# gotaku6629/CTC

Hardware: AMD Instinct MI355X
Metric: ctc_samples_per_sec (higher is better)
Workload: dtype f32; 1 GPU; NoBlankCTC B=256 T=150 C=158 S<=20 fp32 (BASELINE configs[1]); variant=noblank, per_gpu_batch=256, global_batch=256, T=150, C=158, S=20, parallelism=dp1 (batch-sharded), launch=graph, graph_steps=50, step=fused loss+grad launch + scale_grad launch (loss.backward(), grad_out=1)

## Files before the change

### ctc_amd/csrc/noblank_r16.hpp

```cpp
#pragma once

namespace ctc {

typedef float f2_t __attribute__((ext_vector_type(2)));

#define CTC_ROW16(OP)                                                                   \
    "s_nop 1\n\t" OP " %0, %0, %0 quad_perm:[1,0,3,2] row_mask:0xf bank_mask:0xf\n\t"   \
    "s_nop 1\n\t" OP " %0, %0, %0 quad_perm:[2,3,0,1] row_mask:0xf bank_mask:0xf\n\t"   \
    "s_nop 1\n\t" OP " %0, %0, %0 row_half_mirror row_mask:0xf bank_mask:0xf\n\t"       \
    "s_nop 1\n\t" OP " %0, %0, %0 row_mirror row_mask:0xf bank_mask:0xf\n\t"            \
    "s_nop 1"
__device__ __forceinline__ void row16_allmax(float &v) { asm volatile(CTC_ROW16("v_max_f32_dpp") : "+v"(v)); }
__device__ __forceinline__ void row16_allsum(float &v) { asm volatile(CTC_ROW16("v_add_f32_dpp") : "+v"(v)); }
__device__ __forceinline__ void row16_allmax(int &v) { asm volatile(CTC_ROW16("v_max_i32_dpp") : "+v"(v)); }

constexpr int kR16Pad = 2 * kPrefetch + 1;
#ifndef CTC_R16_BLOCK
#define CTC_R16_BLOCK 16
#endif
constexpr int kR16Block = CTC_R16_BLOCK;
__host__ __device__ inline int r16_pitch(int T)
{
    int tp = T + 2 * kR16Pad + 1;
    while ((tp & 3) != 2) ++tp;
    return tp;
}

__device__ __forceinline__ int r16_row(int T, int u, int g, int k)
{
    const int H = (T + 1) >> 1, idx = 2 * kPipeWorkers * g + 2 * u + (k >> 1);
    if ((k & 1) == 0) return idx < H ? idx : -1;
    return idx < T - H ? T - 1 - idx : -1;
}

struct R16Smem {
    int TP;
    cell_t *em, *al, *be;
    float *dummy, *stage, *cs;
    int *cnt, *lab, *occ, *done;
    __device__ R16Smem(float *base, int T, int SP, int RP)
    {
        TP = r16_pitch(T);
        cell_t *lat = reinterpret_cast<cell_t *>(base);
        em = lat + kR16Pad;
        al = em + (size_t)(SP + 1) * TP;
        be = al + (size_t)(SP + 1) * TP;
        dummy = reinterpret_cast<float *>(lat + (size_t)3 * (SP + 1) * TP);
        cnt = reinterpret_cast<int *>(dummy + 8);
        lab = cnt + 16;
        occ = lab + ((SP + 3) & ~3);
        cs = reinterpret_cast<float *>(occ + ((SP + 3) & ~3) + 4);
        done = reinterpret_cast<int *>(cs + 4 * kPipeWorkers);
        stage = cs + 64;
    }
};

static size_t r16_smem_bytes(int T, int SP, int C)
{
    const int RP = 32 * ((C + 31) / 32);
    return (size_t)3 * (SP + 1) * r16_pitch(T) * 8 + (8 + 16 + 2 * ((SP + 3) & ~3) + 4 + 64) * 4 +
           (size_t)kPipeWorkers * 4 * RP * 4;
}

template <bool FWD>
__device__ __forceinline__ cell_t r16_chain(const NoblankParams &p, const R16Smem &sm, int T, int Tb, int L, int SP, const int lane)
{
    constexpr int G = kPipeRows / 4;
    constexpr int D = FWD ? 1 : -1;
    const int lrow = lane < SP ? lane : SP;
    const cell_t *erow = sm.em + (size_t)lrow * sm.TP;
    cell_t *orow = (FWD ? sm.al : sm.be) + (size_t)lrow * sm.TP;
    typedef float pair_t __attribute__((ext_vector_type(4)));
    float m;
    int k;

    const int H = (T + 1) >> 1;
    const int pos0 = FWD ? 0 : T - Tb;
    const int own = FWD ? H : T - H;
    typedef const volatile __attribute__((address_space(3))) int lds_cvint;
    const int *cp = sm.cnt + (lane < kPipeWorkers ? lane : 0);
    int have = 0;
    bool starved = false;
    auto wait_upto = [&](int i_last) {
        const int q = pos0 + (i_last < Tb ? i_last : Tb - 1);
        int ng = q / (2 * kPipeWorkers) + 1;
        if (q >= own || ng > G) ng = G;
        if (ng <= have) return;
        const int need = lane < kPipeWorkers ? 4 * ng : 0;
        int spins = 0;
        while (__builtin_amdgcn_ballot_w64(*(lds_cvint *)cp < need) != 0) {
            if (++spins >= kSpinLimit) { starved = true; break; }
            __builtin_amdgcn_s_sleep(1);
        }
        lds_order();
        have = ng;
    };
#define CTC_R16_STEP_ASM(K, M, EM, EK, K2, T2, DPP)                                                  \
            "v_max_i32_dpp %[kk], " K ", " K " " DPP "\n\t"                                           \
            "v_add_u32 " K2 ", %[kk], " EK "\n\t"                                                     \
            "v_sub_u32 %[d1], " K ", %[kk]\n\t"                                                       \
            "v_sub_u32_dpp %[d2], " K ", %[kk] " DPP "\n\t"                                           \
            "v_ldexp_f32 %[d1], " EM ", %[d1]\n\t"                                                    \
            "v_ldexp_f32 %[d2], " EM ", %[d2]\n\t"                                                    \
            "v_mul_f32 " T2 ", " M ", %[d1]\n\t"                                                      \
            "v_fmac_f32_dpp " T2 ", " M ", %[d2] " DPP "\n\t"
#ifdef CTC_X_ROWDPP
#define CTC_R16_DPP_F "row_shr:1 row_mask:0xf bank_mask:0xf bound_ctrl:1"
#define CTC_R16_DPP_B "row_shl:1 row_mask:0xf bank_mask:0xf bound_ctrl:1"
#else
#define CTC_R16_DPP_F "wave_shr:1 row_mask:0xf bank_mask:0xf bound_ctrl:1"
#define CTC_R16_DPP_B "wave_shl:1 row_mask:0xf bank_mask:0xf bound_ctrl:1"
#endif
    auto step = [&](float em_, float ek_) {
        int kk, k2, d1, d2;
        float t;
        if (FWD)
            asm("s_nop 1\n\t" CTC_R16_STEP_ASM("%[k]", "%[m]", "%[em]", "%[ek]", "%[k2]", "%[t]", CTC_R16_DPP_F)
                : [kk] "=&v"(kk), [k2] "=&v"(k2), [d1] "=&v"(d1), [d2] "=&v"(d2), [t] "=&v"(t)
                : [k] "v"(k), [m] "v"(m), [em] "v"(em_), [ek] "v"(ek_));
        else
            asm("s_nop 1\n\t" CTC_R16_STEP_ASM("%[k]", "%[m]", "%[em]", "%[ek]", "%[k2]", "%[t]", CTC_R16_DPP_B)
                : [kk] "=&v"(kk), [k2] "=&v"(k2), [d1] "=&v"(d1), [d2] "=&v"(d2), [t] "=&v"(t)
                : [k] "v"(k), [m] "v"(m), [em] "v"(em_), [ek] "v"(ek_));
        m = t;
        k = k2;
    };
    auto step2 = [&](pair_t e, bool first) {
        const float e1m = FWD ? e.x : e.z, e1k = FWD ? e.y : e.w, e2m = FWD ? e.z : e.x, e2k = FWD ? e.w : e.y;
        int kk, d1, d2, k1, k2;
        float m1, m2;
#define CTC_R16_PAIR(NOP, DPP)                                                                       \
        asm(NOP CTC_R16_STEP_ASM("%[k]", "%[m]", "%[e1m]", "%[e1k]", "%[k1]", "%[m1]", DPP)           \
                CTC_R16_STEP_ASM("%[k1]", "%[m1]", "%[e2m]", "%[e2k]", "%[k2]", "%[m2]", DPP)         \
            : [kk] "=&v"(kk), [d1] "=&v"(d1), [d2] "=&v"(d2), [k1] "=&v"(k1), [k2] "=&v"(k2),        \
              [m1] "=&v"(m1), [m2] "=&v"(m2)                                                         \
            : [k] "v"(k), [m] "v"(m), [e1m] "v"(e1m), [e1k] "v"(e1k), [e2m] "v"(e2m), [e2k] "v"(e2k))
        if (FWD) { if (first) { CTC_R16_PAIR("s_nop 1\n\t", CTC_R16_DPP_F); } else { CTC_R16_PAIR("", CTC_R16_DPP_F); } }
        else { if (first) { CTC_R16_PAIR("s_nop 1\n\t", CTC_R16_DPP_B); } else { CTC_R16_PAIR("", CTC_R16_DPP_B); } }
#undef CTC_R16_PAIR
        m = m2;
        k = k2;
        const float k1f = __builtin_bit_cast(float, k1), k2f = __builtin_bit_cast(float, k2);
        pair_t o;
        o.x = FWD ? m1 : m2;  o.y = FWD ? k1f : k2f;
        o.z = FWD ? m2 : m1;  o.w = FWD ? k2f : k1f;
        return o;
    };
    auto renorm = [&]() {
        k += __builtin_amdgcn_frexp_expf(m);
        m = __builtin_amdgcn_frexp_mantf(m);
    };

    int *prog = sm.cnt + kPipeWorkers + (FWD ? 0 : 1);
#ifdef CTC_X_NOCHAIN
    *prog = Tb;
    return make_cell(1.f, kXrBias);
#endif
#ifndef CTC_X_NOPRIO
    __builtin_amdgcn_s_setprio(3);
#endif
    wait_upto(kPrefetch + 1);
#ifdef CTC_AMD_FAULT_INJECT
    if (FWD && blockIdx.x == 0) starved = true;
#endif
    int i = 1;
    {
        const int start = FWD ? 0 : L - 1, x = FWD ? 0 : Tb - 1;
        const cell_t e0 = erow[x];
        m = lane == start ? e0.x : 0.f;
        k = lane == start ? kXrBias + cell_k(e0) : 0;
        orow[x] = make_cell(m, k);
        if (!FWD && (Tb & 1) == 1 && Tb > 1) {
            const cell_t e = erow[Tb - 2];
            step(e.x, e.y);
            orow[Tb - 2] = make_cell(m, k);
            i = 2;
        }
    }
    const int x0 = FWD ? i : Tb - 1 - i;
    constexpr int kPairs = kR16Block / 2;
    const pair_t *rb = reinterpret_cast<const pair_t *>(erow + (FWD ? x0 + kPrefetch : x0 - kPrefetch - (kR16Block - 1)));
    pair_t *wb = reinterpret_cast<pair_t *>(orow + (FWD ? x0 : x0 - (kR16Block - 1)));
    pair_t ring[2];
    {
        const pair_t *r0 = reinterpret_cast<const pair_t *>(erow + (FWD ? x0 : x0 - 3));
        ring[0] = r0[FWD ? 0 : 1];
        ring[1] = r0[FWD ? 1 : 0];
    }
    const unsigned long long loop_t0 = CTC_DIAG(p) == -77 ? __builtin_amdgcn_s_memtime() : 0;
    for (; i + kR16Block <= Tb; i += kR16Block) {
        lds_order();
#ifndef CTC_X_NOPROG
        *prog = i;
#endif
        if (have < G) wait_upto(i + kR16Block - 1 + kPrefetch);
        if (CTC_DIAG(p) < 0) stamp(p, 2 + i / 16);
#ifndef CTC_X_NORENORM
        renorm();
#endif
#pragma unroll
        for (int q = 0; q < kPairs; ++q) {
            const pair_t e = ring[q & 1];
#ifndef CTC_X_NOREAD
            ring[q & 1] = rb[FWD ? q : kPairs - 1 - q];
#endif
#ifdef CTC_X_NOWRITE
            const pair_t o = step2(e, q == 0);
            if (q == kPairs - 1) wb[0] = o;
#elif defined(CTC_X_WMASK)
            const pair_t o = step2(e, q == 0);
            if (lane < SP) wb[FWD ? q : kPairs - 1 - q] = o;
#else
            wb[FWD ? q : kPairs - 1 - q] = step2(e, q == 0);
#endif
        }
        rb += D * kPairs;
        wb += D * kPairs;
    }
    if (CTC_DIAG(p) == -77 && lane == 0)
        reinterpret_cast<unsigned long long *>(p.counter)[FWD ? 0 : 1] = __builtin_amdgcn_s_memtime() - loop_t0;
    lds_order();
    *prog = i;
    if (have < G) wait_upto(Tb - 1);
    renorm();
    static_assert(kPrefetch == 4, "tail groups assume one ring revolution of two pairs");
    if (!FWD) { rb += kPairs - 2; wb += kPairs - 2; }
    for (; i < Tb; i += kPrefetch) {
#pragma unroll
        for (int q = 0; q < 2; ++q) {
            const pair_t e = ring[q];
            ring[q] = rb[FWD ? q : 1 - q];
            wb[FWD ? q : 1 - q] = step2(e, q == 0);
        }
        rb += D * 2;
        wb += D * 2;
    }
    lds_order();
    *prog = Tb;
    __builtin_amdgcn_s_setprio(0);
    cell_t fin = (FWD ? sm.al : sm.be)[(size_t)(L - 1) * sm.TP + (FWD ? Tb - 1 : 0)];
    if (starved) {
        raise_status(p.counter, kStatusNoblankStarved);
        fin = make_cell(__builtin_nanf(""), 0);
    }
    return fin;
}

typedef float f4_t __attribute__((ext_vector_type(4)));
typedef float f4u_t __attribute__((ext_vector_type(4), aligned(8)));

typedef unsigned u2a4_t __attribute__((ext_vector_type(2), aligned(4)));
template <typename E>
__device__ __forceinline__ f2_t r16_widen2(unsigned u)
{
    if constexpr (__is_same(E, __bf16)) {
        const f2_t f = {__builtin_bit_cast(float, u << 16), __builtin_bit_cast(float, u & 0xffff0000u)};
        return f;
    } else {
        typedef _Float16 h2_t __attribute__((ext_vector_type(2)));
        return __builtin_convertvector(__builtin_bit_cast(h2_t, u), f2_t);
    }
}
template <typename E>
__device__ __forceinline__ unsigned r16_narrow2(f2_t v)
{
    typedef E e2_t __attribute__((ext_vector_type(2)));
    return __builtin_bit_cast(unsigned, __builtin_convertvector(v, e2_t));
}

template <bool kRaw, int N4, int N2>
struct R16RawRegs {};
template <int N4, int N2>
struct R16RawRegs<true, N4, N2> {
    wt_u2 ra[N4 > 0 ? N4 : 1];
    unsigned rc[N2 > 0 ? N2 : 1];
};

template <int N4, int N2, typename E = float>
struct R16Row : R16RawRegs<sizeof(E) == 2, N4, N2> {
    static constexpr bool kLowp = sizeof(E) == 2;
    f4_t a[N4 > 0 ? N4 : 1];
    f2_t c[N2 > 0 ? N2 : 1];
    static constexpr int kCols = 64 * N4 + 32 * N2;
    static constexpr bool kLast4 = N2 == 0;
    __device__ static __forceinline__ int off4(int j, int i16) { return 64 * j + 4 * i16; }
    __device__ static __forceinline__ int off2(int k, int i16) { return 64 * N4 + 32 * k + 2 * i16; }
    __device__ static __forceinline__ int off_last(int i16) { return kLast4 ? off4(N4 - 1, i16) : off2(N2 - 1, i16); }

    __device__ __forceinline__ void load(const E *row, int i16, int c_last)
    {
        if constexpr (kLowp) {
#pragma unroll
            for (int j = 0; j < N4; ++j)
                this->ra[j] = *reinterpret_cast<const u2a4_t *>(row + ((kLast4 && j == N4 - 1) ? c_last : off4(j, i16)));
#pragma unroll
            for (int k = 0; k < N2; ++k)
                this->rc[k] = *reinterpret_cast<const unsigned *>(row + (k == N2 - 1 ? c_last : off2(k, i16)));
        } else {
#pragma unroll
            for (int j = 0; j < N4; ++j)
                a[j] = *reinterpret_cast<const f4u_t *>(row + ((kLast4 && j == N4 - 1) ? c_last : off4(j, i16)));
#pragma unroll
            for (int k = 0; k < N2; ++k)
                c[k] = *reinterpret_cast<const f2_t *>(row + (k == N2 - 1 ? c_last : off2(k, i16)));
        }
    }
    __device__ __forceinline__ void widen()
    {
        if constexpr (kLowp) {
#pragma unroll
            for (int j = 0; j < N4; ++j) {
                const f2_t lo = r16_widen2<E>(this->ra[j].x), hi = r16_widen2<E>(this->ra[j].y);
                a[j] = f4_t{lo.x, lo.y, hi.x, hi.y};
            }
#pragma unroll
            for (int k = 0; k < N2; ++k) c[k] = r16_widen2<E>(this->rc[k]);
        }
    }
    __device__ __forceinline__ float max() const
    {
        constexpr int n = 4 * N4 + 2 * N2;
        float e[n];
#pragma unroll
        for (int j = 0; j < N4; ++j) { e[4 * j] = a[j].x; e[4 * j + 1] = a[j].y; e[4 * j + 2] = a[j].z; e[4 * j + 3] = a[j].w; }
#pragma unroll
        for (int k = 0; k < N2; ++k) { e[4 * N4 + 2 * k] = c[k].x; e[4 * N4 + 2 * k + 1] = c[k].y; }
        float m = e[0];
#pragma unroll
        for (int i = 1; i + 1 < n; i += 2) m = vmax3(m, e[i], e[i + 1]);
        if ((n & 1) == 0) m = vmax(m, e[n - 1]);
        return m;
    }
    __device__ __forceinline__ float sum(bool valid_last) const
    {
        float s = 0.f;
#pragma unroll
        for (int j = 0; j < N4; ++j) {
            const float q = (a[j].x + a[j].y) + (a[j].z + a[j].w);
            s += ((kLast4 && j == N4 - 1) && !valid_last) ? 0.f : q;
        }
#pragma unroll
        for (int k = 0; k < N2; ++k) s += (k == N2 - 1 && !valid_last) ? 0.f : c[k].x + c[k].y;
        return s;
    }
    __device__ __forceinline__ float exp_sum(float mb, float mbl)
    {
        const f2_t l2 = {kLog2e, kLog2e};
        f2_t acc = {0.f, 0.f};
#pragma unroll
        for (int j = 0; j < N4; ++j) {
            const float b = (kLast4 && j == N4 - 1) ? mbl : mb;
            const f2_t bb = {b, b};
            f2_t lo = {a[j].x, a[j].y}, hi = {a[j].z, a[j].w};
            lo = __builtin_elementwise_fma(lo, l2, bb);
            hi = __builtin_elementwise_fma(hi, l2, bb);
            a[j].x = __builtin_amdgcn_exp2f(lo.x);
            a[j].y = __builtin_amdgcn_exp2f(lo.y);
            a[j].z = __builtin_amdgcn_exp2f(hi.x);
            a[j].w = __builtin_amdgcn_exp2f(hi.y);
            const f2_t e0 = {a[j].x, a[j].y}, e1 = {a[j].z, a[j].w};
            acc += e0;
            acc += e1;
        }
#pragma unroll
        for (int k = 0; k < N2; ++k) {
            const float b = k == N2 - 1 ? mbl : mb;
            const f2_t bb = {b, b};
            const f2_t lo = __builtin_elementwise_fma(c[k], l2, bb);
            c[k].x = __builtin_amdgcn_exp2f(lo.x);
            c[k].y = __builtin_amdgcn_exp2f(lo.y);
            acc += c[k];
        }
        return acc.x + acc.y;
    }
    __device__ __forceinline__ void to_tile(float *trow, int i16) const
    {
#pragma unroll
        for (int j = 0; j < N4; ++j) *reinterpret_cast<f4_t *>(trow + off4(j, i16)) = a[j];
#pragma unroll
        for (int k = 0; k < N2; ++k) *reinterpret_cast<f2_t *>(trow + off2(k, i16)) = c[k];
    }
    __device__ static __forceinline__ void zero_tile(float *trow, int i16)
    {
        const f4_t z4 = {0.f, 0.f, 0.f, 0.f};
        const f2_t z2 = {0.f, 0.f};
#pragma unroll
        for (int j = 0; j < N4; ++j) *reinterpret_cast<f4_t *>(trow + off4(j, i16)) = z4;
#pragma unroll
        for (int k = 0; k < N2; ++k) *reinterpret_cast<f2_t *>(trow + off2(k, i16)) = z2;
    }
    template <bool NT, bool LS>
    __device__ __forceinline__ void store_grad(E *g, const float *trow, int i16, float rs, bool col_ok, float cb) const
    {
        const f2_t r2 = {rs, rs}, cb2 = {cb, cb};
        f4_t o4[N4 > 0 ? N4 : 1];
        f2_t o2[N2 > 0 ? N2 : 1];
#pragma unroll
        for (int j = 0; j < N4; ++j) o4[j] = *reinterpret_cast<const f4_t *>(trow + off4(j, i16));
#pragma unroll
        for (int k = 0; k < N2; ++k) o2[k] = *reinterpret_cast<const f2_t *>(trow + off2(k, i16));
#pragma unroll
        for (int j = 0; j < N4; ++j) {
            const f4_t o = o4[j];
            f2_t olo = {o.x, o.y}, ohi = {o.z, o.w};
            if (LS) { olo += cb2; ohi += cb2; }
            const f2_t xlo = {a[j].x, a[j].y}, xhi = {a[j].z, a[j].w};
            const f2_t vlo = __builtin_elementwise_fma(xlo, r2, olo), vhi = __builtin_elementwise_fma(xhi, r2, ohi);
            if (!(kLast4 && j == N4 - 1) || col_ok) {
                if constexpr (kLowp) {
                    const wt_u2 n = {r16_narrow2<E>(vlo), r16_narrow2<E>(vhi)};
                    grad_store<NT, wt_u2, 4>(reinterpret_cast<wt_u2 *>(g + off4(j, i16)), n);
                } else {
                    const f4_t v = {vlo.x, vlo.y, vhi.x, vhi.y};
                    grad_store<NT>(reinterpret_cast<f4_t *>(g + off4(j, i16)), v);
                }
            }
        }
#pragma unroll
        for (int k = 0; k < N2; ++k) {
            f2_t o = o2[k];
            if (LS) o += cb2;
            const f2_t v = __builtin_elementwise_fma(c[k], r2, o);
            if (k < N2 - 1 || col_ok) {
                if constexpr (kLowp) grad_store<NT, unsigned, 4>(reinterpret_cast<unsigned *>(g + off2(k, i16)), r16_narrow2<E>(v));
                else grad_store<NT>(reinterpret_cast<f2_t *>(g + off2(k, i16)), v);
            }
        }
    }
    __device__ __forceinline__ void touch() const
    {
        if constexpr (kLowp) {
#pragma unroll
            for (int j = 0; j < N4; ++j) asm volatile("" ::"v"(this->ra[j]));
#pragma unroll
            for (int k = 0; k < N2; ++k) asm volatile("" ::"v"(this->rc[k]));
        } else {
#pragma unroll
            for (int j = 0; j < N4; ++j) asm volatile("" ::"v"(a[j]));
#pragma unroll
            for (int k = 0; k < N2; ++k) asm volatile("" ::"v"(c[k]));
        }
    }
    template <bool NT>
    __device__ static __forceinline__ void store_zero(E *g, int i16, bool col_ok)
    {
        if constexpr (kLowp) {
            const wt_u2 z4 = {0u, 0u};
#pragma unroll
            for (int j = 0; j < N4; ++j)
                if (!(kLast4 && j == N4 - 1) || col_ok) grad_store<NT, wt_u2, 4>(reinterpret_cast<wt_u2 *>(g + off4(j, i16)), z4);
#pragma unroll
            for (int k = 0; k < N2; ++k)
                if (k < N2 - 1 || col_ok) grad_store<NT, unsigned, 4>(reinterpret_cast<unsigned *>(g + off2(k, i16)), 0u);
            return;
        }
        const f4_t z4 = {0.f, 0.f, 0.f, 0.f};
        const f2_t z2 = {0.f, 0.f};
#pragma unroll
        for (int j = 0; j < N4; ++j)
            if (!(kLast4 && j == N4 - 1) || col_ok) grad_store<NT>(reinterpret_cast<f4_t *>(g + off4(j, i16)), z4);
#pragma unroll
        for (int k = 0; k < N2; ++k)
            if (k < N2 - 1 || col_ok) grad_store<NT>(reinterpret_cast<f2_t *>(g + off2(k, i16)), z2);
    }
};

static bool r16_shape(int C, int &n4, int &n2)
{
    if (C < 2 || C > 256 || (C & 1)) return false;
    const int U = (C + 31) / 32;
    if (U & 1) { n4 = U / 2; n2 = 1; }
    else if ((C & 3) == 0) { n4 = U / 2; n2 = 0; }
    else { n4 = U / 2 - 1; n2 = 2; }
    return true;
}

template <typename E>
__device__ __forceinline__ const E *r16_xrow(const NoblankParams &p, int t, int b)
{
    return reinterpret_cast<const E *>(p.x) + (int64_t)t * p.st + (int64_t)b * p.sb;
}
template <int N4, int N2, bool NT, bool PS = false, typename E = float>
__global__ __launch_bounds__(kThreads, 4) void noblank_r16_kernel(NoblankParams p)
{
    extern __shared__ float4 smem_raw[];
    typedef R16Row<N4, N2, E> Row;
    constexpr int RP = Row::kCols;
    constexpr int G = kPipeRows / 4;
    const R16Smem sm(reinterpret_cast<float *>(smem_raw), p.T, p.SP, RP);
    const int tid = threadIdx.x, w = wave_id(), lane = lane_id();
    int vb = blockIdx.x;
    int b = xcd_sample(vb, p.B);
    if (tid == 64 * kChainB) note_arrival(p.counter, b);
    const int u = (w == 0 || w == kChainB) ? -1 : (w < kChainB ? w - 1 : w - 2);
    const int rho = lane >> 4, i16 = lane & 15;

    if (CTC_DIAG(p) == 1) return;
    stamp(p, 0);
    stamp_setup(p, 0);
    auto spread = [&](int which) {
        if (CTC_DIAG(p) != -50 || w != 1 || lane != 0) return;
        const int bid = blockIdx.x, nb = gridDim.x;
        const int slot = bid == 0 ? 0 : bid == nb / 2 ? 2 : bid == nb - 1 ? 4 : -1;
        if (slot < 0) return;
        unsigned long long *o = reinterpret_cast<unsigned long long *>(p.counter) + 8 + 2 * (slot + which);
        o[0] = __builtin_amdgcn_s_memtime();
        o[1] = __builtin_amdgcn_s_memrealtime();
    };
    spread(0);
    ScalarLengths len(p.in_len + b, p.tgt_len + b);
    int tv0[G];
    Row v[G];
#ifdef CTC_R16_NX
    constexpr int NX = PS ? CTC_R16_NX : 0;
#else
    constexpr int NX = PS ? (NT ? 2 : 3) : 0;
#endif
    Row nx[NX > 0 ? NX : 1];
    const bool col_ok = Row::off_last(i16) < p.C;
    const int c_last = col_ok ? Row::off_last(i16) : p.C - (Row::kLast4 ? 4 : 2);
    const int Hh = (p.T + 1) >> 1;
    bool grp[G];
#pragma unroll
    for (int g = 0; g < G; ++g) grp[g] = u >= 0 && 2 * kPipeWorkers * g + 2 * u < Hh;
    int klab = 0;
    if (PS && w == 0 && lane < p.S) klab = load_label(p.lab, p.lab64, (int64_t)b * p.S + lane);
    if (u >= 0) {
#pragma unroll
        for (int g = 0; g < G; ++g) {
            tv0[g] = r16_row(p.T, u, g, rho);
            if (g >= NX) v[g].load(r16_xrow<E>(p, tv0[g] >= 0 ? tv0[g] : 0, b), i16, c_last);
            else nx[g].load(r16_xrow<E>(p, tv0[g] >= 0 ? tv0[g] : 0, b), i16, c_last);
        }
        stamp_setup(p, 1);
        if (PS) {
#pragma unroll
            for (int g = 0; g < G; ++g) {
                if (g < NX) nx[g].touch();
                else v[g].touch();
            }
        }
    }
    const float ninf = -__builtin_inff();
    typedef const volatile __attribute__((address_space(3))) int lds_cvint;
    int Tb = 0, L = 0, bn = b, vbn = vb, klab_n = 0;
    bool more = false;
    ScalarLengths len_n;
    const cell_t zero = make_cell(0.f, 0);
    auto begin = [&](const bool chain_role) -> bool {
        int64_t Tb64, L64;
        len.get(Tb64, L64);
        stamp_setup(p, 2);
        const bool ok = L64 >= 1 && L64 <= p.S && Tb64 >= L64 && Tb64 <= p.T;
        Tb = ok ? (int)Tb64 : 0;
        L = ok ? (int)L64 : 0;
        vbn = vb + (int)gridDim.x;
        more = PS && vbn < p.B;
        bn = more ? xcd_sample(vbn, p.B) : b;
        if (PS) len_n = ScalarLengths(p.in_len + bn, p.tgt_len + bn);
        klab_n = 0;
        if (chain_role && w == 0) {
            int k = 0;
            if (lane < L) {
                k = (PS ? klab : load_label(p.lab, p.lab64, (int64_t)b * p.S + lane)) % p.C;
                if (k < 0) k += p.C;
            }
            if (lane < p.SP) sm.lab[lane] = k;
            if (more && lane < p.S) klab_n = load_label(p.lab, p.lab64, (int64_t)bn * p.S + lane);
        }
        stamp_setup(p, 3);
        for (int i = tid; i < (p.SP + 1) * sm.TP; i += kThreads) sm.em[i - kR16Pad] = zero;
        if (tid < 16) sm.cnt[tid] = 0;
        if (tid == 16) *sm.done = 0;
        if (tid == 17) sm.occ[((p.SP + 3) & ~3) + 1] = 0;
        if (tid < 8) sm.dummy[tid] = 0.f;
        stamp_setup(p, 4);
        asm volatile("s_waitcnt lgkmcnt(0)\n\ts_barrier" ::: "memory");
        stamp(p, 1);
        stamp_setup(p, 5);
        stamp_mode(p, -200, (vb - (int)blockIdx.x) / (int)gridDim.x);
        if ((vb - (int)blockIdx.x) / (int)gridDim.x < 6) stamp_mode(p, -400, (vb - (int)blockIdx.x) / (int)gridDim.x);
        return CTC_DIAG(p) != 2;
    };
    auto advance = [&]() -> bool {
        stamp_mode(p, -300, (vb - (int)blockIdx.x) / (int)gridDim.x);
        if ((vb - (int)blockIdx.x) / (int)gridDim.x < 6) stamp_mode(p, -400, 6 + (vb - (int)blockIdx.x) / (int)gridDim.x);
        if (!more) return false;
        vb = vbn;
        b = bn;
        len = len_n;
        klab = klab_n;
        asm volatile("s_waitcnt lgkmcnt(0)\n\ts_barrier" ::: "memory");
        return true;
    };
    auto chain_sample = [&](const NoblankParams &p, const int lane) {
    const R16Smem sm(reinterpret_cast<float *>(smem_raw), p.T, p.SP, RP);
    if (Tb == 0) {
        if (w == 0)
            publish_and_reduce_sum(-kNeg, b, p.B, p.nll, p.loss, p.loss_scale, p.counter);
        return;
    }
    {
        __builtin_amdgcn_s_setprio(3);
        if (w == 0) {
            const cell_t a = r16_chain<true>(p, sm, p.T, Tb, L, p.SP, lane);
            stamp(p, 11);
            bool late = false;
            {
                int spins = 0;
                while (*(lds_cvint *)sm.done < kPipeWorkers) {
                    if (++spins >= kSpinLimit) { late = true; break; }
                    __builtin_amdgcn_s_sleep(2);
                }
                lds_order();
            }
            const float csum = wave_sum(lane < 4 * kPipeWorkers ? sm.cs[lane] : 0.f);
            const float am = a.x;
            float nll = am > 0.f ? -(__builtin_amdgcn_logf(am) + (float)(cell_k(a) - kXrBias) + csum) * kLn2 : -kNeg;
            if (am != am) nll = am;
            if (late) {
                raise_status(p.counter, kStatusNoblankStarved);
                nll = __builtin_nanf("");
            }
            publish_and_reduce_sum(nll, b, p.B, p.nll, p.loss, p.loss_scale, p.counter);
            if (CTC_DIAG(p) == -50 && lane == 0) {
                const int bid = blockIdx.x, nb = gridDim.x;
                const int slot = bid == 0 ? 6 : bid == nb / 2 ? 7 : bid == nb - 1 ? 8 : -1;
                if (slot >= 0) {
                    unsigned long long *o = reinterpret_cast<unsigned long long *>(p.counter) + 8 + 2 * slot;
                    o[0] = __builtin_amdgcn_s_memtime();
                    o[1] = __builtin_amdgcn_s_memrealtime();
                }
            }
        } else if (p.grad || p.gamma) {
            r16_chain<false>(p, sm, p.T, Tb, L, p.SP, lane);
            stamp(p, 11);
        }
    }
    };

    auto worker_sample = [&](const NoblankParams &p, const int lane, const int u) {
    const R16Smem sm(reinterpret_cast<float *>(smem_raw), p.T, p.SP, RP);
    const int rho = lane >> 4, i16 = lane & 15;
    int tv[G];
#pragma unroll
    for (int g = 0; g < G; ++g) tv[g] = PS ? opaque_v(tv0[g]) : tv0[g];
    const bool has_grad = PS || p.grad != nullptr, has_gamma = !PS && !Row::kLowp && p.gamma != nullptr;
    auto load_next = [&]() {
        if (!PS) return;
#pragma unroll
        for (int g = 0; g < NX; ++g) nx[g].load(r16_xrow<E>(p, tv[g] >= 0 ? tv[g] : 0, bn), i16, c_last);
    };
#define CTC_R16_RELOAD(g)                                                                             \
    do {                                                                                              \
        if (PS && (g) >= NX) v[g].load(r16_xrow<E>(p, tv[g] >= 0 ? tv[g] : 0, bn), i16, c_last); \
    } while (0)
    if (!PS && Tb == 0) {
        if (p.grad) {
#pragma unroll
            for (int g = 0; g < G; ++g)
                if (tv[g] >= 0) Row::template store_zero<NT>(reinterpret_cast<E *>(p.grad) + ((int64_t)tv[g] * p.B + b) * p.C, i16, col_ok);
        }
        if (!Row::kLowp && p.gamma) {
#pragma unroll
            for (int g = 0; g < G; ++g)
                for (int l = i16; l < p.S && tv[g] >= 0; l += 16) p.gamma[((int64_t)b * p.T + tv[g]) * p.S + l] = 0.f;
        }
        return;
    }
    float *tile = sm.stage + (size_t)u * 4 * RP;
    float *trow = tile + rho * RP;
    int lst[2];
    float *gat[2];
#pragma unroll
    for (int s = 0; s < 2; ++s) {
        lst[s] = 16 * s + i16;
        gat[s] = trow + (lst[s] < p.SP ? sm.lab[lst[s]] : 0);
    }
    const bool own[2] = {lst[0] < L, lst[1] < L};
    const bool smooth = p.ls_b != 0.f;
    cell_t *const spare_w = reinterpret_cast<cell_t *>(sm.dummy);
    float mrow[G];
#pragma unroll
    for (int g = 0; g < G; ++g) {
        if (g == 0) __builtin_amdgcn_s_setprio(2);
        else __builtin_amdgcn_s_setprio(1);
        if (g < NX) v[g] = nx[g];
        if (grp[g]) {
            Row &x = v[g];
            x.widen();
            const int t = tv[g];
            const bool live = t >= 0 && t < Tb;
            float m = x.max();
            row16_allmax(m);
            mrow[g] = m;
            if (CTC_DIAG(p) < 0 && g == 0) stamp(p, 6);
            x.to_tile(trow, i16);
            lds_order();
            float xv[2];
#pragma unroll
            for (int s = 0; s < 2; ++s) xv[s] = *gat[s];
            lds_order();
#pragma unroll
            for (int s = 0; s < 2; ++s) {
                const float ec = (xv[s] - m) * kLog2e;
                const float e2 = fmaxf(smooth ? p.ls_a * ec : ec, kXrMinLog2);
                const float fl = __builtin_floorf(e2);
                const float pm = __builtin_amdgcn_exp2f(e2 - fl);
                cell_t *dst = (live && lst[s] < p.SP) ? sm.em + lst[s] * sm.TP + t : spare_w;
                *dst = own[s] ? make_cell(pm, (int)fl) : zero;
            }
            lds_order();
        } else {
            mrow[g] = 0.f;
        }
        sm.cnt[u] = 4 * (g + 1);
        __builtin_amdgcn_sched_barrier(0);
        if (CTC_DIAG(p) < 0) stamp(p, 8 + g);
    }
    __builtin_amdgcn_s_setprio(0);
    load_next();
    float rs[G];
    float cacc = 0.f;
#pragma unroll
    for (int g = 0; g < G; ++g) {
        rs[g] = 0.f;
        if (!grp[g]) continue;
        Row &x = v[g];
        const int t = tv[g];
        const bool live = t >= 0 && t < Tb;
        const float m = mrow[g];
        float sx = 0.f;
        if (smooth) {
            sx = x.sum(col_ok);
            row16_allsum(sx);
        }
        const float mb = -m * kLog2e;
        float sum = x.exp_sum(mb, col_ok ? mb : ninf);
        row16_allsum(sum);
        const float l2sum = __builtin_amdgcn_logf(sum);
        rs[g] = live ? p.grad_scale * __builtin_amdgcn_rcpf(sum) : 0.f;
        const float cst = smooth ? __builtin_fmaf(p.ls_b, __builtin_fmaf(sx - (float)p.C * m, kLog2e, -(float)p.C * l2sum), -p.ls_a * l2sum)
                                 : -l2sum;
        cacc += live ? cst : 0.f;
    }
    if (i16 == 0) sm.cs[4 * u + rho] = cacc;
    lds_order();
    if (lane == 0) __hip_atomic_fetch_add(sm.done, 1, __ATOMIC_RELAXED, __HIP_MEMORY_SCOPE_WORKGROUP);
    stamp(p, 2);
    if (u == kPipeWorkers - 1 && has_grad) {
        const int kl = lane < p.SP ? sm.lab[lane] : -1;
        int oc = 0;
        for (int l2 = 0; l2 < L; ++l2) {
            const int q = __builtin_amdgcn_readlane(kl, l2);
            oc += (l2 < lane && q == kl) ? 1 : 0;
        }
        if (lane >= L) oc = 0;
        int mo = 0;
        while (__builtin_amdgcn_ballot_w64(oc > mo) != 0) ++mo;
        if (lane < p.SP) sm.occ[lane] = oc;
        sm.occ[(p.SP + 3) & ~3] = mo;
        lds_order();
        sm.occ[((p.SP + 3) & ~3) + 1] = 1;
    }
    float prefetched = 0.f;
    if (!PS && p.next_round > 0 && (int)blockIdx.x + p.next_round < p.B) {
        const int nb = xcd_sample(blockIdx.x + p.next_round, p.B);
        const int line = u * kWave + lane;
        const int lines_per_row = (p.C * (int)sizeof(E) + 127) / 128;
        const int t = line / lines_per_row, c = (line - t * lines_per_row) * (128 / (int)sizeof(E));
        typedef const E __attribute__((address_space(1))) gelem;
        if (t < p.T) prefetched = (float)*(gelem *)(r16_xrow<E>(p, t, nb) + (c < p.C ? c : p.C - 1));
    }
    if (!has_grad && !has_gamma) return;

    const int Tlive = Tb;
    const float gsc = p.grad_scale;
    Row::zero_tile(trow, i16);
    lds_order();
    if (PS) {
#pragma unroll
        for (int g = 0; g < NX; ++g) nx[g].touch();
    }
    int need_a_[G], need_b_[G];
#pragma unroll
    for (int g = 0; g < G; ++g) {
        need_a_[g] = 0;
        need_b_[g] = 0;
#pragma unroll
        for (int k = 0; k < 4; ++k) {
            const int tk = r16_row(p.T, u, g, k);
            if (tk >= 0 && tk < Tlive) {
                need_a_[g] = max(need_a_[g], tk + 1);
                need_b_[g] = max(need_b_[g], Tlive - tk);
            }
        }
    }
    int crow[2];
#pragma unroll
    for (int s = 0; s < 2; ++s) crow[s] = opaque_v((lst[s] < p.SP ? lst[s] : p.SP) * sm.TP);
    E *grow[G];
#pragma unroll
    for (int g = 0; g < G; ++g) {
        grow[g] = reinterpret_cast<E *>(p.grad) + ((int64_t)(tv[g] > 0 ? tv[g] : 0) * p.B + b) * p.C;
        asm volatile("" : "+v"(grow[g]));
    }
    bool starved = false;

    int kref = 0;
    bool have_ref = false;
    int occn[2] = {0, 0}, max_occ = 0;
    if (has_grad) {
        int spins = 0;
        while (*(lds_cvint *)(sm.occ + ((p.SP + 3) & ~3) + 1) == 0) {
            if (++spins >= kSpinLimit) { starved = true; break; }
            __builtin_amdgcn_s_sleep(2);
        }
        lds_order();
        occn[0] = own[0] ? sm.occ[lst[0]] : 0;
        occn[1] = own[1] ? sm.occ[lst[1]] : 0;
        max_occ = __builtin_amdgcn_readfirstlane(sm.occ[(p.SP + 3) & ~3]);
    }
    const bool first_occ[2] = {own[0] && occn[0] == 0, own[1] && occn[1] == 0};
    float *const sink = sm.dummy + 4;
#pragma unroll
    for (int g = G - 1; g >= 0; --g) {
        if (!grp[g]) continue;
        const int need_a = need_a_[g], need_b = need_b_[g];
        if (need_a > 0) {
            int spins = 0;
            while (*(lds_cvint *)(sm.cnt + kPipeWorkers) < need_a || *(lds_cvint *)(sm.cnt + kPipeWorkers + 1) < need_b) {
                if (++spins >= kSpinLimit) { starved = true; break; }
                __builtin_amdgcn_s_sleep(8);
            }
            lds_order();
        }
#ifdef CTC_AMD_FAULT_INJECT
        if (b == 1) starved = true;
#endif
        if (CTC_DIAG(p) < 0) stamp(p, 3 + (G - 1 - g));
        if (g == G - 1) asm volatile("" ::"v"(prefetched));
        const Row &x = v[g];
        const int t = tv[g];
        const bool live = t >= 0 && t < Tlive;
        float pr[2];
        int ks[2];
#pragma unroll
        for (int s = 0; s < 2; ++s) {
            const bool in = live && own[s];
            const int off = crow[s] + (t > 0 ? t : 0);
            const cell_t a = sm.al[off], bb = sm.be[off], e = sm.em[off];
            pr[s] = in ? a.x * bb.x * __builtin_amdgcn_rcpf(e.x) : 0.f;
            ks[s] = cell_k(a) + cell_k(bb) - cell_k(e);
        }
        if (__builtin_amdgcn_ballot_w64(live && !have_ref) != 0) {
            int km = max(pr[0] > 0.f ? ks[0] : 0, pr[1] > 0.f ? ks[1] : 0);
            row16_allmax(km);
            if (live && !have_ref) { kref = km; have_ref = true; }
        }
        float z[2];
#pragma unroll
        for (int s = 0; s < 2; ++s) z[s] = __builtin_amdgcn_ldexpf(pr[s], ks[s] - kref);
        float tot = z[0] + z[1];
        row16_allsum(tot);
        if (has_gamma) {
            const float ginv = (live && tot > 0.f) ? __builtin_amdgcn_rcpf(tot) : 0.f;
#pragma unroll
            for (int s = 0; s < 2; ++s)
                if (t >= 0 && lst[s] < p.S) p.gamma[((int64_t)b * p.T + t) * p.S + lst[s]] = own[s] ? z[s] * ginv : 0.f;
            continue;
        }
        float rinv = (live && tot > 0.f) ? -gsc * p.ls_a * __builtin_amdgcn_rcpf(tot) : 0.f;
        if (starved) {
            rinv = __builtin_nanf("");
            raise_status(p.counter, kStatusNoblankStarved);
        }
#pragma unroll
        for (int s = 0; s < 2; ++s) *(first_occ[s] ? gat[s] : sink) = z[s] * rinv;
        for (int k = 1; k <= max_occ; ++k) {
            lds_order();
#pragma unroll
            for (int s = 0; s < 2; ++s)
                if (own[s] && occn[s] == k) *gat[s] += z[s] * rinv;
        }
        lds_order();
        if (t >= 0) {
            E *gp = grow[g];
            if (smooth) x.template store_grad<NT, true>(gp, trow, i16, rs[g] * (1.f - p.ls_b), col_ok, live ? -p.ls_b * gsc : 0.f);
            else x.template store_grad<NT, false>(gp, trow, i16, rs[g], col_ok, 0.f);
        }
        lds_order();
#pragma unroll
        for (int s = 0; s < 2; ++s) *(own[s] ? gat[s] : sink) = 0.f;
        lds_order();
        CTC_R16_RELOAD(g);
    }
    stamp(p, 7);
    spread(1);
#undef CTC_R16_RELOAD
    };

    if (u < 0) {
        for (;;) {
            if (!begin(true)) return;
            chain_sample(p, PS ? opaque_v(lane) : lane);
            if (!advance()) return;
        }
    }
    for (;;) {
        if (!begin(false)) return;
        if (PS) worker_sample(p, opaque_v(lane), opaque_s(u));
        else worker_sample(p, lane, u);
        if (!advance()) return;
    }
}

#ifdef CTC_AMD_DIAGNOSTICS
__global__ __launch_bounds__(kThreads, 4) void r16_chain_probe_kernel(NoblankParams p, unsigned long long *out, int waves_alive,
                                                                     int mode, int chain_b)
{
    extern __shared__ float4 smem_raw[];
    const R16Smem sm(reinterpret_cast<float *>(smem_raw), p.T, p.SP, 160);
    const int tid = threadIdx.x, w = wave_id(), lane = lane_id();
    for (int i = tid; i < 3 * (p.SP + 1) * sm.TP; i += kThreads) sm.em[i - kR16Pad] = make_cell(1.5f, -1);
    if (tid < 16) sm.cnt[tid] = kPipeRows;
    __syncthreads();
    if (w >= waves_alive && w != chain_b) return;
    if (w != 0 && w != chain_b) {
        typedef const volatile __attribute__((address_space(3))) int lds_cvint;
        int spins = 0;
        const int u = (w < chain_b ? w - 1 : w - 2) % kPipeWorkers;
        float *tile = sm.stage + (size_t)u * 4 * 160 + (lane >> 4) * 160 + 4 * (lane & 15);
        const cell_t *cells = sm.al + (size_t)(lane & 15) * sm.TP;
        if (mode & 8) __builtin_amdgcn_s_setprio(2);
        float a0 = lane, a1 = 1.f, a2 = 2.f, a3 = 3.f, acc = 0.f;
        const int kind = mode & 7;
        while (*(lds_cvint *)(sm.cnt + kPipeWorkers) < p.T && ++spins < 100000) {
            if (kind == 0) { __builtin_amdgcn_s_sleep(8); continue; }
            if (kind & 1) {
#pragma unroll
                for (int r = 0; r < 16; ++r) {
                    a0 = __builtin_fmaf(a0, 1.0001f, a1); a1 = __builtin_fmaf(a1, 0.9999f, a2);
                    a2 = __builtin_fmaf(a2, 1.0001f, a3); a3 = __builtin_fmaf(a3, 0.9999f, a0);
                    a0 = __builtin_fmaf(a0, 0.5f, a2); a1 = __builtin_fmaf(a1, 0.5f, a3);
                    a2 = __builtin_fmaf(a2, 0.5f, 1.f);
                    a3 = __builtin_amdgcn_exp2f(a3 * 1e-3f);
                }
            }
            if (kind & 2) {
                const int reps = kind == 2 ? 12 : 1;
                for (int r = 0; r < reps; ++r) {
                    f4_t v4 = {a0, a1, a2, a3};
                    *reinterpret_cast<f4_t *>(tile) = v4;
                    *reinterpret_cast<f4_t *>(tile + 64) = v4;
                    *reinterpret_cast<f2_t *>(tile + 128) = f2_t{a0, a1};
                    lds_order();
                    const f4_t r4 = *reinterpret_cast<const f4_t *>(tile + 64);
                    const cell_t c0 = cells[8 + (spins & 63)], c1 = cells[sm.TP * 16 + 9 + (spins & 63)];
                    acc += r4.x + c0.x + c1.x;
                    lds_order();
                }
            }
        }
        if (acc + a0 + a1 + a2 + a3 == 12345.f) out[15] = 1;
        return;
    }
    const unsigned long long t0 = __builtin_amdgcn_s_memtime();
    const cell_t c = w == 0 ? r16_chain<true>(p, sm, p.T, p.T, p.SP, p.SP, lane) : r16_chain<false>(p, sm, p.T, p.T, p.SP, p.SP, lane);
    const unsigned long long t1 = __builtin_amdgcn_s_memtime();
    if (lane == 0 && blockIdx.x == 0) {
        out[w == 0 ? 0 : 1] = t1 - t0;
        out[4 + (w == 0 ? 0 : 1)] = (unsigned long long)cell_k(c);
    }
}
#endif

}
```

Baseline: 19.30 million samples/s.

## Track producer frontier per position and fall back to small groups when starved

Result: no change. 19.48 million samples/s, median of 6 (+0.9%).

```diff
diff --git a/ctc_amd/csrc/noblank_r16.hpp b/ctc_amd/csrc/noblank_r16.hpp
--- a/ctc_amd/csrc/noblank_r16.hpp
+++ b/ctc_amd/csrc/noblank_r16.hpp
@@ -79,21 +79,39 @@
     const int own = FWD ? H : T - H;
     typedef const volatile __attribute__((address_space(3))) int lds_cvint;
     const int *cp = sm.cnt + (lane < kPipeWorkers ? lane : 0);
-    int have = 0;
+    constexpr int kAll = 1 << 30;
+    int F = 0;
     bool starved = false;
-    auto wait_upto = [&](int i_last) {
+    static_assert(2 * kPipeWorkers == 28, "28 (c / 4) = 8 c - c below");
+    const int lane2 = lane < kPipeWorkers ? 2 * lane : 0;
+    auto look = [&](int q) {
+        const int c = *(lds_cvint *)cp;
+        const int f = c >= 4 * G ? kAll : ((c << 3) - c) + lane2;
+        if (__builtin_amdgcn_ballot_w64(f <= q) == 0) {
+            int nf = -f;
+            row16_allmax(nf);
+            F = -__builtin_amdgcn_readfirstlane(nf);
+        }
+        lds_order();
+    };
+    auto last_pos = [&](int i_last) {
         const int q = pos0 + (i_last < Tb ? i_last : Tb - 1);
-        int ng = q / (2 * kPipeWorkers) + 1;
-        if (q >= own || ng > G) ng = G;
-        if (ng <= have) return;
-        const int need = lane < kPipeWorkers ? 4 * ng : 0;
+        return q >= own ? kAll - 1 : q;
+    };
+    auto ready = [&](int i_last) {
+        const int q = last_pos(i_last);
+        if (q >= F) look(q);
+        return q < F;
+    };
+    auto wait_ready = [&](int i_last) {
+        const int q = last_pos(i_last);
         int spins = 0;
-        while (__builtin_amdgcn_ballot_w64(*(lds_cvint *)cp < need) != 0) {
-            if (++spins >= kSpinLimit) { starved = true; break; }
+        while (q >= F) {
+            look(q);
+            if (q < F) break;
+            if (++spins >= kSpinLimit) { starved = true; F = kAll; break; }
             __builtin_amdgcn_s_sleep(1);
         }
-        lds_order();
-        have = ng;
     };
 #define CTC_R16_STEP_ASM(K, M, EM, EK, K2, T2, DPP)                                                  \
             "v_max_i32_dpp %[kk], " K ", " K " " DPP "\n\t"                                           \
@@ -129,12 +147,36 @@
         const float e1m = FWD ? e.x : e.z, e1k = FWD ? e.y : e.w, e2m = FWD ? e.z : e.x, e2k = FWD ? e.w : e.y;
         int kk, d1, d2, k1, k2;
         float m1, m2;
+#ifdef CTC_X_PAIR_ILV
+        int kk2, d3, d4;
+#define CTC_R16_PAIR(NOP, DPP)                                                                       \
+        asm(NOP "v_max_i32_dpp %[kk], %[k], %[k] " DPP "\n\t"                                         \
+                "v_add_u32 %[k1], %[kk], %[e1k]\n\t"                                                  \
+                "v_sub_u32 %[d1], %[k], %[kk]\n\t"                                                    \
+                "v_sub_u32_dpp %[d2], %[k], %[kk] " DPP "\n\t"                                        \
+                "v_max_i32_dpp %[kk2], %[k1], %[k1] " DPP "\n\t"                                      \
+                "v_ldexp_f32 %[d1], %[e1m], %[d1]\n\t"                                                \
+                "v_ldexp_f32 %[d2], %[e1m], %[d2]\n\t"                                                \
+                "v_add_u32 %[k2], %[kk2], %[e2k]\n\t"                                                 \
+                "v_mul_f32 %[m1], %[m], %[d1]\n\t"                                                    \
+                "v_sub_u32 %[d3], %[k1], %[kk2]\n\t"                                                  \
+                "v_fmac_f32_dpp %[m1], %[m], %[d2] " DPP "\n\t"                                       \
+                "v_sub_u32_dpp %[d4], %[k1], %[kk2] " DPP "\n\t"                                      \
+                "v_ldexp_f32 %[d3], %[e2m], %[d3]\n\t"                                                \
+                "v_ldexp_f32 %[d4], %[e2m], %[d4]\n\t"                                                \
+                "v_mul_f32 %[m2], %[m1], %[d3]\n\t"                                                   \
+                "v_fmac_f32_dpp %[m2], %[m1], %[d4] " DPP "\n\t"                                      \
+            : [kk] "=&v"(kk), [d1] "=&v"(d1), [d2] "=&v"(d2), [k1] "=&v"(k1), [k2] "=&v"(k2),        \
+              [m1] "=&v"(m1), [m2] "=&v"(m2), [kk2] "=&v"(kk2), [d3] "=&v"(d3), [d4] "=&v"(d4)       \
+            : [k] "v"(k), [m] "v"(m), [e1m] "v"(e1m), [e1k] "v"(e1k), [e2m] "v"(e2m), [e2k] "v"(e2k))
+#else
 #define CTC_R16_PAIR(NOP, DPP)                                                                       \
         asm(NOP CTC_R16_STEP_ASM("%[k]", "%[m]", "%[e1m]", "%[e1k]", "%[k1]", "%[m1]", DPP)           \
                 CTC_R16_STEP_ASM("%[k1]", "%[m1]", "%[e2m]", "%[e2k]", "%[k2]", "%[m2]", DPP)         \
             : [kk] "=&v"(kk), [d1] "=&v"(d1), [d2] "=&v"(d2), [k1] "=&v"(k1), [k2] "=&v"(k2),        \
               [m1] "=&v"(m1), [m2] "=&v"(m2)                                                         \
             : [k] "v"(k), [m] "v"(m), [e1m] "v"(e1m), [e1k] "v"(e1k), [e2m] "v"(e2m), [e2k] "v"(e2k))
+#endif
         if (FWD) { if (first) { CTC_R16_PAIR("s_nop 1\n\t", CTC_R16_DPP_F); } else { CTC_R16_PAIR("", CTC_R16_DPP_F); } }
         else { if (first) { CTC_R16_PAIR("s_nop 1\n\t", CTC_R16_DPP_B); } else { CTC_R16_PAIR("", CTC_R16_DPP_B); } }
 #undef CTC_R16_PAIR
@@ -159,41 +201,39 @@
 #ifndef CTC_X_NOPRIO
     __builtin_amdgcn_s_setprio(3);
 #endif
-    wait_upto(kPrefetch + 1);
+    const bool peel = !FWD && (Tb & 1) == 1 && Tb > 1;
+    int i = peel ? 2 : 1;
+    const int x0 = FWD ? i : Tb - 1 - i;
+    wait_ready(i + kPrefetch - 1);
 #ifdef CTC_AMD_FAULT_INJECT
     if (FWD && blockIdx.x == 0) starved = true;
 #endif
-    int i = 1;
+    pair_t ring[2];
     {
         const int start = FWD ? 0 : L - 1, x = FWD ? 0 : Tb - 1;
+        const pair_t *r0 = reinterpret_cast<const pair_t *>(erow + (FWD ? x0 : x0 - 3));
         const cell_t e0 = erow[x];
+        const cell_t e1 = erow[peel ? Tb - 2 : x];
+        ring[0] = r0[FWD ? 0 : 1];
+        ring[1] = r0[FWD ? 1 : 0];
         m = lane == start ? e0.x : 0.f;
         k = lane == start ? kXrBias + cell_k(e0) : 0;
         orow[x] = make_cell(m, k);
-        if (!FWD && (Tb & 1) == 1 && Tb > 1) {
-            const cell_t e = erow[Tb - 2];
-            step(e.x, e.y);
+        if (peel) {
+            step(e1.x, e1.y);
             orow[Tb - 2] = make_cell(m, k);
-            i = 2;
-        }
-    }
-    const int x0 = FWD ? i : Tb - 1 - i;
+        }
+    }
     constexpr int kPairs = kR16Block / 2;
-    const pair_t *rb = reinterpret_cast<const pair_t *>(erow + (FWD ? x0 + kPrefetch : x0 - kPrefetch - (kR16Block - 1)));
-    pair_t *wb = reinterpret_cast<pair_t *>(orow + (FWD ? x0 : x0 - (kR16Block - 1)));
-    pair_t ring[2];
-    {
-        const pair_t *r0 = reinterpret_cast<const pair_t *>(erow + (FWD ? x0 : x0 - 3));
-        ring[0] = r0[FWD ? 0 : 1];
-        ring[1] = r0[FWD ? 1 : 0];
-    }
+    static_assert(kPrefetch == 4 && kR16Block % kPrefetch == 0, "groups of one ring revolution of two pairs");
+    const pair_t *rb = reinterpret_cast<const pair_t *>(erow + (FWD ? x0 + kPrefetch : x0 - kPrefetch - (kPrefetch - 1)));
+    pair_t *wb = reinterpret_cast<pair_t *>(orow + (FWD ? x0 : x0 - (kPrefetch - 1)));
     const unsigned long long loop_t0 = CTC_DIAG(p) == -77 ? __builtin_amdgcn_s_memtime() : 0;
-    for (; i + kR16Block <= Tb; i += kR16Block) {
+    auto block = [&]() {
         lds_order();
 #ifndef CTC_X_NOPROG
         *prog = i;
 #endif
-        if (have < G) wait_upto(i + kR16Block - 1 + kPrefetch);
         if (CTC_DIAG(p) < 0) stamp(p, 2 + i / 16);
 #ifndef CTC_X_NORENORM
         renorm();
@@ -216,24 +256,49 @@
         }
         rb += D * kPairs;
         wb += D * kPairs;
-    }
-    if (CTC_DIAG(p) == -77 && lane == 0)
-        reinterpret_cast<unsigned long long *>(p.counter)[FWD ? 0 : 1] = __builtin_amdgcn_s_memtime() - loop_t0;
-    lds_order();
-    *prog = i;
-    if (have < G) wait_upto(Tb - 1);
-    renorm();
-    static_assert(kPrefetch == 4, "tail groups assume one ring revolution of two pairs");
-    if (!FWD) { rb += kPairs - 2; wb += kPairs - 2; }
-    for (; i < Tb; i += kPrefetch) {
-#pragma unroll
-        for (int q = 0; q < 2; ++q) {
-            const pair_t e = ring[q];
-            ring[q] = rb[FWD ? q : 1 - q];
-            wb[FWD ? q : 1 - q] = step2(e, q == 0);
-        }
-        rb += D * 2;
-        wb += D * 2;
+        i += kR16Block;
+    };
+    for (;;) {
+        if (i + kR16Block <= Tb && ready(i + kR16Block - 1 + kPrefetch)) {
+            if (!FWD) { rb -= kPairs - 2; wb -= kPairs - 2; }
+            bool go = true;
+            while (go && F != kAll) {
+                block();
+                go = i + kR16Block <= Tb && ready(i + kR16Block - 1 + kPrefetch);
+            }
+            if (go) {
+                do block();
+                while (i + kR16Block <= Tb);
+            }
+            if (!FWD) { rb += kPairs - 2; wb += kPairs - 2; }
+            if (CTC_DIAG(p) == -77 && lane == 0)
+                reinterpret_cast<unsigned long long *>(p.counter)[FWD ? 0 : 1] = __builtin_amdgcn_s_memtime() - loop_t0;
+        }
+        lds_order();
+        *prog = i;
+        if (CTC_DIAG(p) < 0 && i < Tb) stamp(p, 2 + i / 16);
+        renorm();
+        auto group = [&]() {
+#pragma unroll
+            for (int q = 0; q < 2; ++q) {
+                const pair_t e = ring[q];
+                ring[q] = rb[FWD ? q : 1 - q];
+                wb[FWD ? q : 1 - q] = step2(e, q == 0);
+            }
+            rb += D * 2;
+            wb += D * 2;
+            i += kPrefetch;
+        };
+        if (F == kAll && i + kR16Block > Tb) {
+            while (i < Tb) group();
+            break;
+        }
+        const int i_end = i + kR16Block < Tb ? i + kR16Block : Tb;
+        while (i < i_end) {
+            wait_ready(i + 2 * kPrefetch - 1);
+            group();
+        }
+        if (i >= Tb) break;
     }
     lds_order();
     *prog = Tb;
```
